# SakodaShintaro/f2-nerf

Measured on AMD Instinct MI355X. Metric: rendered rays/sec (fwd+bwd) at 800x800, higher is better.
Workload: dtype f32; 1 GPU; ngp_fox-like synthetic views 800x800, 128 samples/ray, L=16 F=2 T=2^19, 65536-ray chunks, TRAIN render + loss + backward (optimizer excluded); pixel_order=rows, regime=dense

## Files before the change

### f2-nerf_amd/csrc/host/bindings.cpp

```cpp
#include <torch/extension.h>

#include "fused_adam.hpp"
#include "hash_3d_anchored.hpp"
#include "kernel_timer.hpp"
#include "localizer.hpp"
#include "occupancy_grid.hpp"
#include "points_sampler.hpp"
#include "ragged_ops.hpp"
#include "rays.hpp"
#include "scene_files.hpp"
#include "renderer.hpp"
#include "sh_shader.hpp"

namespace py = pybind11;
using torch::Tensor;

namespace
{

torch::Device parse_device(const std::string & s)
{
  return s.empty() ? f2n::default_device() : torch::Device(s);
}

// ... 159 lines not shown
        o.step = step;
        return std::make_shared<PtsSampler>(o);
      }),
      py::arg("max_samples") = MAX_SAMPLE_PER_RAY, py::arg("step") = 1.0f / 256)
    .def(
      "get_samples",
      [](PtsSampler & s, const Tensor & o, const Tensor & d, const std::string & mode,
         const c10::optional<Tensor> & noise) {
        SampleResultFlex r = noise.has_value() ? s.get_samples(o, d, *noise)
                                               : s.get_samples(o, d, parse_mode(mode));
        return py::make_tuple(r.pts, r.dirs, r.dt, r.t, r.pts_idx_bounds);
      },
      py::arg("rays_o"), py::arg("rays_d"), py::arg("mode") = "validate",
      py::arg("noise") = py::none())
    .def(
      "get_samples_aten",
      [](PtsSampler & s, const Tensor & o, const Tensor & d, const c10::optional<Tensor> & noise) {
        SampleResultFlex r = s.get_samples_aten(o, d, opt_tensor(noise));
        return py::make_tuple(r.pts, r.dirs, r.dt, r.t, r.pts_idx_bounds);
      },
      py::arg("rays_o"), py::arg("rays_d"), py::arg("noise") = py::none());

  py::class_<SHShader, std::shared_ptr<SHShader>>(m, "SHShader")
    .def(
      py::init([](const std::string & dev) { return std::make_shared<SHShader>(parse_device(dev)); }),
      py::arg("device") = "")
    .def("query", &SHShader::query)
    .def("encode", &SHShader::encode)
    .def("named_parameters", [](SHShader & s) { return named_params(s); });

// ... 100 lines not shown
        for (auto & kv : r.named_parameters()) d[py::str(kv.key())] = grad_or_none(kv.value());
        return d;
      })
    .def(
      "set_occupancy",
      [](Renderer & r, std::shared_ptr<OccupancyGrid> g) { r.set_occupancy(std::move(g)); },
      py::arg("grid").none(true), "attach an occupancy grid (None = off): see Renderer::set_occupancy")
    .def_property_readonly("occupancy", [](Renderer & r) { return r.occupancy(); })
    .def("set_fused", [](Renderer & r, bool f) { r.options_.fused = f; })
    .def("set_fused_shade", [](Renderer & r, bool f) { r.options_.fused_shade = f; })
    .def("set_dense_first_pass", [](Renderer & r, int m) { r.options_.dense_first_pass = m; })
    .def("set_speculate_dense", [](Renderer & r, bool f) { r.options_.speculate_dense = f; })
    .def("set_pixel_tiles", [](Renderer & r, int b) { r.options_.pixel_tiles = b; })
    .def("set_fused_ray_grad", [](Renderer & r, bool f) { r.options_.fused_ray_grad = f; },
         "rays that require grad take the fused path: see RendererOptions::fused_ray_grad")
    .def("set_margin_min_samples", [](Renderer & r, int64_t n) { r.options_.margin_min_samples = n; })
    .def("set_one_pass", &Renderer::set_one_pass,
         "render_all_rays / render_image in one kernel per chunk: see RendererOptions::one_pass")
    .def("one_pass_applies", &Renderer::one_pass_applies)
    .def_property_readonly(
      "one_pass_head", [](const Renderer & r) { return r.options_.one_pass_head; },
      "RendererOptions::one_pass_head as set_one_pass_head left it")
    .def("set_one_pass_head", &Renderer::set_one_pass_head,
         "how the one-pass render walks a ray: 0 one wavefront per ray (default), -1 whole rays eight "
         "to a wavefront, a positive multiple of 64 = head then tail; see RendererOptions::one_pass_head")
    .def("set_deferred_check", [](Renderer & r, bool f) { r.options_.deferred_check = f; },
         "no host read in render(): see RendererOptions::deferred_check")
    .def("deferred_check_ok", &Renderer::deferred_check_ok)
    .def_readonly("last_kept_fraction", &Renderer::last_kept_fraction_)
    .def_readonly("last_n_samples", &Renderer::last_n_samples_)
// ... 174 lines not shown
```

### f2-nerf_amd/csrc/host/hash_3d_anchored.cpp

```cpp
#include "hash_3d_anchored.hpp"

#include "kernel_timer.hpp"

#include <cmath>

#include <c10/hip/HIPGuard.h>
#include <hip/hip_runtime_api.h>

using Tensor = torch::Tensor;

TORCH_LIBRARY(dec_hash3d_anchored, m)
{
  m.class_<Hash3DAnchoredInfo>("Hash3DAnchoredInfo").def(torch::init());
}

namespace
{

class ContractFn : public torch::autograd::Function<ContractFn>
{
public:
  static torch::autograd::variable_list forward(torch::autograd::AutogradContext * ctx, Tensor points)
  {
    points = f2n::dev_f32(points, "Hash3DAnchored::query points");
// ... 131 lines not shown
          prim_pool_.data_ptr<int32_t>(),
          bias_pool_.data_ptr<float>(),
          level_mul_.data_ptr<float>(),
          (int)options_.n_levels,
          (int)options_.n_channels,
          (uint32_t)local_size_,
          level_stride_};
}

std::pair<Tensor, Tensor> Hash3DAnchored::density_head() const
{
  return {mlp_->weight.detach().select(0, 0).contiguous(),
          mlp_->bias.detach().slice(0, 0, 1).contiguous()};
}

Tensor Hash3DAnchored::encode(const Tensor & points, int64_t samples_per_ray, Tensor * contracted_out)
{
  auto info = torch::make_intrusive<Hash3DAnchoredInfo>();
  info->hash3d_ = this;
  info->samples_per_ray_ = samples_per_ray;

  Tensor x = ContractFn::apply(points)[0];
  if (contracted_out) *contracted_out = x.detach();
  return torch::autograd::Hash3DAnchoredFunction::apply(x, feat_pool_, torch::IValue(info))[0];
}

Tensor Hash3DAnchored::encode_cached(
  const Tensor & points, const Tensor & enc_cm, const Tensor & contracted)
{
  TORCH_CHECK(
    enc_cm.dim() == 2 && enc_cm.is_contiguous() && enc_cm.size(1) == points.size(0) &&
      enc_cm.size(0) == options_.n_levels * options_.n_channels,
    "encode_cached: enc_cm must be contiguous [L*F, n]");
  auto info = torch::make_intrusive<Hash3DAnchoredInfo>();
  info->hash3d_ = this;
  info->precomputed_cm_ = enc_cm;
  const bool reuse = contracted.defined() && contracted.sizes() == points.sizes() &&
// ... 136 lines not shown
```

### f2-nerf_amd/csrc/host/hash_3d_anchored.hpp

```cpp
#pragma once

#include "common.hpp"

struct Hash3DAnchoredOptions
{
  int64_t n_levels = 16;
  int64_t n_channels = 2;
  int64_t log2_table = 19;
  int64_t level_stride = 0;
  int64_t mlp_out_dim = 16;
  bool binned_backward = true;
  bool accumulate_in_place = true;
  torch::Device device = f2n::default_device();
};

namespace f2n
{

struct FieldArgs
{
  const uint16_t * table;
  const int32_t * primes;
  const float *bias, *mul;
  int L, F;
  uint32_t T;
  int64_t level_stride;
};

}

class Hash3DAnchored : public torch::nn::Module
{
  using Tensor = torch::Tensor;

public:
  explicit Hash3DAnchored(const Hash3DAnchoredOptions & opt = {});

  Tensor query(const Tensor & points);

  Tensor encode(const Tensor & points, int64_t samples_per_ray = 0, Tensor * contracted_out = nullptr);

  Tensor encode_cached(
    const Tensor & points, const Tensor & enc_cm, const Tensor & contracted = Tensor());

  std::pair<Tensor, Tensor> density_head() const;

  Tensor table_f16();
  Tensor table_for(const Tensor & feat_pool);
  f2n::FieldArgs kernel_args(const Tensor & table16) const;

  Tensor shadow_storage();
  void mark_shadow_fresh();

  std::vector<torch::optim::OptimizerParamGroup> optim_param_groups(float lr);

// ... 40 lines not shown
```

### f2-nerf_amd/csrc/host/points_sampler.cpp

```cpp
#include "points_sampler.hpp"

using Tensor = torch::Tensor;

PtsSampler::PtsSampler(const PtsSamplerOptions & opt) : options_(opt)
{
  TORCH_CHECK(opt.max_samples >= 1 && opt.step > 0.f, "PtsSampler: bad options");
}

Tensor PtsSampler::draw_noise(int64_t n_rays, RunningMode mode, const torch::Device & device) const
{
  if (mode == RunningMode::VALIDATE) return Tensor();
  return ((torch::rand({n_rays, (int64_t)options_.max_samples}, f2n::float_on(device)) - .5f) + 1.f)
    .contiguous();
}

SampleResultFlex PtsSampler::get_samples(
  const Tensor & rays_o, const Tensor & rays_d, RunningMode mode)
{
  return get_samples(rays_o, rays_d, draw_noise(rays_o.size(0), mode, rays_o.device()));
}

SampleResultFlex PtsSampler::get_samples(
  const Tensor & rays_o_raw, const Tensor & rays_d_raw, const Tensor & noise_raw)
{
  Tensor rays_o = f2n::dev_f32(rays_o_raw, "rays_o");
  Tensor rays_d = f2n::dev_f32(rays_d_raw, "rays_d");
  const int n_rays = (int)rays_o.size(0);
  const int S = options_.max_samples;
  const int64_t n_all = (int64_t)n_rays * S;
  Tensor noise;
  if (noise_raw.defined()) {
    noise = f2n::dev_f32(noise_raw, "noise");
    TORCH_CHECK(noise.numel() == n_all, "noise must hold n_rays * max_samples values");
  }
  const auto fopt = rays_o.options();
  SampleResultFlex res;
  res.pts = torch::empty({n_all, 3}, fopt);
  res.dirs = torch::empty({n_all, 3}, fopt);
  res.dt = torch::empty({n_all}, fopt);
  res.t = torch::empty({n_all}, fopt);
  res.pts_idx_bounds = torch::empty({n_rays, 2}, f2n::int_on(rays_o.device()));
  f2n::check(
    f2n_sample_rays(
      rays_o.data_ptr<float>(), rays_d.data_ptr<float>(), f2n::fptr(noise),
      res.pts.data_ptr<float>(), res.dirs.data_ptr<float>(), res.dt.data_ptr<float>(),
      res.t.data_ptr<float>(), res.pts_idx_bounds.data_ptr<int32_t>(), n_rays, S, options_.step,
      f2n::current_stream(rays_o)),
    "f2n_sample_rays");
  return res;
}

SampleResultFlex PtsSampler::get_samples_aten(
  const Tensor & rays_o_raw, const Tensor & rays_d_raw, const Tensor & noise_raw)
{
  const int64_t S = options_.max_samples;
  Tensor rays_o = rays_o_raw.contiguous();
// ... 18 lines not shown
```

### f2-nerf_amd/csrc/host/points_sampler.hpp

```cpp
#pragma once

#include "common.hpp"

constexpr int MAX_SAMPLE_PER_RAY = 1024;

struct SampleResultFlex
{
  using Tensor = torch::Tensor;
  Tensor pts;
  Tensor dirs;
  Tensor dt;
  Tensor t;
  Tensor pts_idx_bounds;
};

enum RunningMode { TRAIN, VALIDATE };

struct PtsSamplerOptions
{
  int max_samples = MAX_SAMPLE_PER_RAY;
  float step = 1.0f / 256;
};

class PtsSampler
{
  using Tensor = torch::Tensor;

public:
  explicit PtsSampler(const PtsSamplerOptions & opt = {});

  SampleResultFlex get_samples(const Tensor & rays_o, const Tensor & rays_d, RunningMode mode);
  SampleResultFlex get_samples(const Tensor & rays_o, const Tensor & rays_d, const Tensor & noise);

  SampleResultFlex get_samples_aten(
    const Tensor & rays_o, const Tensor & rays_d, const Tensor & noise);

  Tensor draw_noise(int64_t n_rays, RunningMode mode, const torch::Device & device) const;

  PtsSamplerOptions options_;
};
```

### f2-nerf_amd/csrc/host/ragged_ops.cpp

```cpp
#include "ragged_ops.hpp"

#include "kernel_timer.hpp"

using torch::Tensor;
using torch::autograd::AutogradContext;
using torch::autograd::variable_list;

namespace
{

class FlexSumFn : public torch::autograd::Function<FlexSumFn>
{
public:
  static variable_list forward(AutogradContext * ctx, Tensor val, Tensor idx)
  {
    val = f2n::dev_f32(val, "FlexOps::Sum val");
    idx = f2n::dev_i32(idx, "FlexOps::Sum idx_start_end");
    TORCH_CHECK(val.dim() == 1 || val.dim() == 2, "FlexOps::Sum expects [n] or [n, c]");
    const int n_rays = (int)idx.size(0);
    void * s = f2n::current_stream(val);
    Tensor sum;
    if (val.dim() == 1) {
      sum = torch::empty({n_rays}, val.options());
      f2n::check(
// ... 151 lines not shown
  {
    field_out = f2n::dev_f32(field_out, "composite field_out");
    rgb = f2n::dev_f32(rgb, "composite rgb");
    dt = f2n::dev_f32(dt, "composite dt");
    t = f2n::dev_f32(t, "composite t");
    idx = f2n::dev_i32(idx, "composite idx_start_end");
    bg = f2n::dev_f32(bg, "composite bg_color");
    TORCH_CHECK(field_out.dim() == 2 && rgb.dim() == 2 && rgb.size(1) == 3, "composite shapes");
    const int64_t n = field_out.size(0);
    const int n_rays = (int)idx.size(0);
    auto opt = field_out.options();
    Tensor colors = torch::empty({n_rays, 3}, opt), depths = torch::empty({n_rays}, opt);
    Tensor weights = tiled ? torch::empty({n}, opt) : torch::zeros({n}, opt);
    Tensor last_trans = torch::empty({n_rays}, opt);
    ctx->saved_data["tiled"] = tiled;
    f2n::check(
      f2n_composite_fwd(
        f2n::fptr(field_out), field_out.size(1), f2n::fptr(rgb), f2n::fptr(dt), f2n::fptr(t),
        f2n::iptr(idx), f2n::fptr(bg), colors.data_ptr<float>(), depths.data_ptr<float>(),
        weights.data_ptr<float>(), last_trans.data_ptr<float>(), n_rays, 3.f, 1e-2f,
        f2n::current_stream(field_out)),
      "f2n_composite_fwd");
    ctx->save_for_backward({field_out, rgb, dt, t, idx, bg, weights, last_trans});
    return {colors, depths, weights};
  }

  static variable_list backward(AutogradContext * ctx, variable_list grad_output)
  {
    auto sv = ctx->get_saved_variables();
    Tensor &field_out = sv[0], &rgb = sv[1], &dt = sv[2], &t = sv[3], &idx = sv[4], &bg = sv[5],
// ... 12 lines not shown
    Tensor d_rgb = tiled ? torch::empty({n, 3}, opt) : torch::zeros({n, 3}, opt);
    f2n::check(
      f2n_composite_bwd(
        f2n::fptr(field_out), field_out.size(1), f2n::fptr(rgb), f2n::fptr(dt), f2n::fptr(t),
        f2n::iptr(idx), f2n::fptr(bg), f2n::fptr(weights), f2n::fptr(last_trans),
        f2n::fptr(d_colors), f2n::fptr(d_depths), f2n::fptr(d_weights), d_logit.data_ptr<float>(),
        d_rgb.data_ptr<float>(), n_rays, 3.f, 1e-2f, f2n::current_stream(field_out)),
      "f2n_composite_bwd");
    if (field_out.size(1) == 1)
      return {d_logit.unsqueeze(1), d_rgb, Tensor(), Tensor(), Tensor(), Tensor(), Tensor()};
    Tensor d_field = torch::zeros_like(field_out);
    d_field.select(1, 0).copy_(d_logit);
    return {d_field, d_rgb, Tensor(), Tensor(), Tensor(), Tensor(), Tensor()};
  }
};

Tensor as_channel_major(const Tensor & t)
{
  if (t.dim() == 2 && t.stride(0) == 1 && t.stride(1) == t.size(0)) return t.t();
  return t.t().contiguous();
}

class ShadeFn : public torch::autograd::Function<ShadeFn>
{
public:
  static variable_list forward(
    AutogradContext * ctx, Tensor enc, Tensor dirs, Tensor sample_img, Tensor w_h, Tensor b_h,
    Tensor w1, Tensor b1, Tensor w2, Tensor b2, Tensor app_emb)
  {
    TORCH_CHECK(enc.is_cuda() && enc.scalar_type() == torch::kFloat32 && enc.dim() == 2, "enc");
// ... 34 lines not shown

  static variable_list backward(AutogradContext * ctx, variable_list grad_output)
  {
    auto sv = ctx->get_saved_variables();
    Tensor &enc_cm = sv[0], &dirs = sv[1], &sample_img = sv[2], &w_h = sv[3], &b_h = sv[4],
           &w1 = sv[5], &b1 = sv[6], &w2 = sv[7], &b2 = sv[8], &emb = sv[9];
    const int C = (int)enc_cm.size(0);
    const int64_t n = enc_cm.size(1);
    auto opt = enc_cm.options();
    Tensor d_logit = grad_output[0].defined() ? f2n::dev_f32(grad_output[0], "d_logit")
                                              : torch::zeros({n}, opt);
    Tensor d_rgb = grad_output[1].defined() ? f2n::dev_f32(grad_output[1], "d_rgb")
                                            : torch::zeros({n, 3}, opt);
    Tensor d_enc_cm = torch::empty({(int64_t)C, n}, opt);
    const bool use_emb = emb.defined() && sample_img.defined();
    auto pad4 = [](int64_t v) { return (v + 3) / 4 * 4; };
    const int64_t sizes[7] = {w_h.numel(), b_h.numel(), w1.numel(), b1.numel(),
                              w2.numel(), b2.numel(), use_emb ? emb.numel() : 0};
    int64_t total = 0;
    for (int64_t v : sizes) total += pad4(v);
    Tensor gbuf = torch::zeros({total}, opt);
    int64_t off = 0;
    auto take = [&](const Tensor & like, int64_t numel) {
      Tensor v = gbuf.narrow(0, off, numel).view(like.sizes());
      off += pad4(numel);
      return v;
    };
    Tensor g_w_h = take(w_h, sizes[0]), g_b_h = take(b_h, sizes[1]), g_w1 = take(w1, sizes[2]),
           g_b1 = take(b1, sizes[3]), g_w2 = take(w2, sizes[4]), g_b2 = take(b2, sizes[5]);
    Tensor g_emb = use_emb ? take(emb, sizes[6]) : Tensor();
    {
    f2n::ScopedKernelTimer timer("shade_bwd", f2n::current_stream(enc_cm), (double)n);
    f2n::check(
      f2n_shade_bwd(
        enc_cm.data_ptr<float>(), C, dirs.data_ptr<float>(), use_emb ? f2n::iptr(sample_img) : nullptr,
        f2n::fptr(w_h), f2n::fptr(b_h), f2n::fptr(w1), f2n::fptr(b1), f2n::fptr(w2), f2n::fptr(b2),
        f2n::fptr(emb), f2n::fptr(d_logit), f2n::fptr(d_rgb), d_enc_cm.data_ptr<float>(),
        g_w_h.data_ptr<float>(), g_b_h.data_ptr<float>(), g_w1.data_ptr<float>(),
        g_b1.data_ptr<float>(), g_w2.data_ptr<float>(), g_b2.data_ptr<float>(),
        use_emb ? g_emb.data_ptr<float>() : nullptr, nullptr, n,
        f2n::current_stream(enc_cm)),
      "f2n_shade_bwd");
    }
    return {d_enc_cm.t(), Tensor(), Tensor(), g_w_h, g_b_h, g_w1, g_b1, g_w2, g_b2, g_emb};
  }
};

class ShadeRaysFn : public torch::autograd::Function<ShadeRaysFn>
{
public:
  static variable_list forward(
    AutogradContext * ctx, Tensor enc, Tensor dirs, Tensor ray_img, int64_t S, Tensor w_h,
    Tensor b_h, Tensor w1, Tensor b1, Tensor w2, Tensor b2, Tensor app_emb)
  {
    TORCH_CHECK(enc.is_cuda() && enc.scalar_type() == torch::kFloat32 && enc.dim() == 2, "enc");
    const int64_t n = enc.size(0);
    const int C = (int)enc.size(1);
    TORCH_CHECK(S > 0 && S % 64 == 0 && n % S == 0 && n < ((int64_t)1 << 28), "shade_rays: n = n_rays * S, S % 64 == 0");
    const int n_rays = (int)(n / S);
// ... 36 lines not shown

  static variable_list backward(AutogradContext * ctx, variable_list grad_output)
  {
    auto sv = ctx->get_saved_variables();
    Tensor &enc_cm = sv[0], &dirs = sv[1], &ray_img = sv[2], &w_h = sv[3], &b_h = sv[4],
           &w1 = sv[5], &b1 = sv[6], &w2 = sv[7], &b2 = sv[8], &emb = sv[9];
    const int C = (int)enc_cm.size(0);
    const int64_t n = enc_cm.size(1), S = ctx->saved_data["S"].toInt();
    auto opt = enc_cm.options();
    Tensor d_logit = grad_output[0].defined() ? f2n::dev_f32(grad_output[0], "d_logit")
                                              : torch::zeros({n}, opt);
    Tensor d_rgb = grad_output[1].defined() ? f2n::dev_f32(grad_output[1], "d_rgb")
                                            : torch::zeros({n, 3}, opt);
    Tensor d_enc_cm = torch::empty({(int64_t)C, n}, opt);
    const bool use_emb = emb.defined() && ray_img.defined();
    auto pad4 = [](int64_t v) { return (v + 3) / 4 * 4; };
    const int64_t sizes[7] = {w_h.numel(), b_h.numel(), w1.numel(), b1.numel(),
                              w2.numel(), b2.numel(), use_emb ? emb.numel() : 0};
    int64_t total = 0;
    for (int64_t v : sizes) total += pad4(v);
    Tensor gbuf = torch::zeros({total}, opt);
    int64_t off = 0;
    auto take = [&](const Tensor & like, int64_t numel) {
      Tensor v = gbuf.narrow(0, off, numel).view(like.sizes());
      off += pad4(numel);
      return v;
    };
    Tensor g_w_h = take(w_h, sizes[0]), g_b_h = take(b_h, sizes[1]), g_w1 = take(w1, sizes[2]),
           g_b1 = take(b1, sizes[3]), g_w2 = take(w2, sizes[4]), g_b2 = take(b2, sizes[5]);
    Tensor g_emb = use_emb ? take(emb, sizes[6]) : Tensor();
    {
    f2n::ScopedKernelTimer timer("shade_bwd", f2n::current_stream(enc_cm), (double)n);
    f2n::check(
      f2n_shade_bwd_rays(
        enc_cm.data_ptr<float>(), C, dirs.data_ptr<float>(), use_emb ? f2n::iptr(ray_img) : nullptr,
        f2n::fptr(w_h), f2n::fptr(b_h), f2n::fptr(w1), f2n::fptr(b1), f2n::fptr(w2), f2n::fptr(b2),
        f2n::fptr(emb), f2n::fptr(d_logit), f2n::fptr(d_rgb), d_enc_cm.data_ptr<float>(),
        g_w_h.data_ptr<float>(), g_b_h.data_ptr<float>(), g_w1.data_ptr<float>(),
        g_b1.data_ptr<float>(), g_w2.data_ptr<float>(), g_b2.data_ptr<float>(),
        use_emb ? g_emb.data_ptr<float>() : nullptr, (int)(n / S), (int)S,
        f2n::current_stream(enc_cm)),
      "f2n_shade_bwd_rays");
    }
    return {d_enc_cm.t(), Tensor(), Tensor(), Tensor(), g_w_h, g_b_h, g_w1, g_b1, g_w2, g_b2, g_emb};
  }
};


class TrainLossFn : public torch::autograd::Function<TrainLossFn>
{
public:
  static variable_list forward(
    AutogradContext * ctx, Tensor colors, Tensor gt, Tensor var, double var_weight)
  {
    colors = f2n::dev_f32(colors, "train_loss colors");
    gt = f2n::dev_f32(gt, "train_loss gt_colors");
    var = f2n::dev_f32(var, "train_loss var");
    const int64_t n_rays = colors.size(0);
    TORCH_CHECK(
// ... 105 lines not shown
bool f2n::shade_rays_applies(int64_t n, int64_t n_rays, int64_t S)
{
  return n_rays > 0 && S > 0 && S % 64 == 0 && n == n_rays * S && n < ((int64_t)1 << 28) &&
         f2n_get_option(F2N_OPT_SHADE_RAYS) == 0 && f2n_get_option(F2N_OPT_SHADE_FWD) == 0 &&
         f2n_get_option(F2N_OPT_SHADE_BWD) == 0;
}

f2n::CompositeOut f2n::composite(
  const Tensor & field_out, const Tensor & rgb, const Tensor & dt, const Tensor & t,
  const Tensor & idx_start_end, const Tensor & bg_color, bool bounds_tile_samples)
{
  auto out = CompositeFn::apply(field_out, rgb, dt, t, idx_start_end, bg_color, bounds_tile_samples);
  return {out[0], out[1], out[2]};
}

Tensor f2n::train_loss(
  const Tensor & colors, const Tensor & gt_colors, const Tensor & var, float var_loss_weight)
{
  return TrainLossFn::apply(colors, gt_colors, var, (double)var_loss_weight)[0];
}
```

### f2-nerf_amd/csrc/host/ragged_ops.hpp

```cpp
#pragma once

#include "common.hpp"

namespace torch::autograd
{

class TruncExp : public Function<TruncExp>
{
public:
  static variable_list forward(AutogradContext * ctx, Tensor input);
  static variable_list backward(AutogradContext * ctx, variable_list grad_output);
};

}

namespace FlexOps
{
torch::Tensor Sum(torch::Tensor val, torch::Tensor idx_start_end);
torch::Tensor AccumulateSum(torch::Tensor val, torch::Tensor idx_start_end, bool include_this);
}

namespace CustomOps
{
torch::Tensor WeightVar(torch::Tensor weights, torch::Tensor idx_start_end);
// ... 25 lines not shown
ShadeOut shade(
  const Tensor & enc, const Tensor & dirs, const Tensor & sample_img, const Tensor & w_h,
  const Tensor & b_h, const Tensor & w1, const Tensor & b1, const Tensor & w2, const Tensor & b2,
  const Tensor & app_emb);

ShadeOut shade_rays(
  const Tensor & enc, const Tensor & dirs, const Tensor & ray_img, int64_t S, const Tensor & w_h,
  const Tensor & b_h, const Tensor & w1, const Tensor & b1, const Tensor & w2, const Tensor & b2,
  const Tensor & app_emb);

bool shade_rays_applies(int64_t n, int64_t n_rays, int64_t S);

Tensor train_loss(
  const Tensor & colors, const Tensor & gt_colors, const Tensor & var, float var_loss_weight);

inline bool shade_supported(int64_t C) { return C == 8 || C == 16 || C == 32 || C == 64; }

}
```

### f2-nerf_amd/csrc/host/renderer.cpp

```cpp
#include "renderer.hpp"

#include "kernel_timer.hpp"

#include "ragged_ops.hpp"
#include "rays.hpp"

#include <c10/hip/HIPGuard.h>
#include <hip/hip_runtime_api.h>

using Tensor = torch::Tensor;

f2n::HostCount::~HostCount()
{
  if (event_) hipEventDestroy((hipEvent_t)event_);
  if (pinned_) hipHostFree(pinned_);
}

void f2n::HostCount::request(const torch::Tensor & device_int32, void * stream)
{
  TORCH_CHECK(
    device_int32.is_cuda() && device_int32.scalar_type() == torch::kInt32 && device_int32.numel() == 1,
    "HostCount: one int32 on the device");
  const int device = (int)device_int32.device().index();
  c10::hip::HIPGuard on_device(device);
// ... 46 lines not shown
class RayUnpermuteFn : public torch::autograd::Function<RayUnpermuteFn>
{
public:
  static torch::autograd::variable_list forward(
    torch::autograd::AutogradContext * ctx, Tensor colors, Tensor depths, Tensor weights,
    Tensor perm, Tensor inv, Tensor bounds_sorted, Tensor bounds_caller, int64_t S, bool rows)
  {
    colors = f2n::dev_f32(colors, "colors");
    depths = f2n::dev_f32(depths, "depths");
    weights = f2n::dev_f32(weights, "weights");
    const int n = (int)perm.size(0);
    void * s = f2n::current_stream(colors);
    Tensor c = torch::empty_like(colors), d = torch::empty_like(depths), w = torch::empty_like(weights);
    gather(colors, depths, weights, c, d, w, inv, bounds_sorted, bounds_caller, n, S, rows, s);
    ctx->save_for_backward({perm, bounds_sorted, bounds_caller});
    ctx->saved_data["S"] = S;
    ctx->saved_data["rows"] = rows;
    return {c, d, w};
  }

  static torch::autograd::variable_list backward(
    torch::autograd::AutogradContext * ctx, torch::autograd::variable_list g)
  {
    auto saved = ctx->get_saved_variables();
    const Tensor & perm = saved[0];
    const int n = (int)perm.size(0);
    const int64_t S = ctx->saved_data["S"].toInt();
    const bool rows = ctx->saved_data["rows"].toBool();
    Tensor gc = g[0].defined() ? f2n::dev_f32(g[0], "grad colors") : Tensor();
    Tensor gd = g[1].defined() ? f2n::dev_f32(g[1], "grad depths") : Tensor();
// ... 332 lines not shown
    bounds = bounds_from_counts(counts, stream).first;
  }
  auto out = RayUnpermuteFn::apply(
    r.colors, r.depths, r.weights, perm, inv, r.idx_start_end, bounds, S, rows);
  return {out[0], out[1], out[2], bounds};
}

RenderResult Renderer::render_dense(
  const Tensor & rays_o, const Tensor & rays_d, const Tensor & emb_idx, RunningMode mode,
  const Tensor & noise, const Tensor & bg_color, const Route & route)
{
  const int n_rays = (int)rays_o.size(0);
  const int S = pts_sampler_->options_.max_samples;
  void * stream = f2n::current_stream(rays_o);
  Hash3DAnchored & field = *scene_field_;
  SampleResultFlex all = pts_sampler_->get_samples(rays_o, rays_d, noise);
  const int64_t n_all = all.pts.size(0);
  Tensor contracted_all, enc_all_cm;
  {
    torch::NoGradGuard no_grad;
    enc_all_cm = field.encode(all.pts, S, &contracted_all).t();
    TORCH_CHECK(enc_all_cm.is_contiguous(), "encode() must return channel-major storage");
  }

  if (options_.deferred_check) {
    Tensor total = scan_survivors(all, enc_all_cm, n_rays).second;
    if (!deferred_bad_.defined()) deferred_bad_ = torch::zeros({1}, total.options());
    deferred_bad_.add_(total.ne(n_all).to(torch::kInt32));
    record_kept(n_all, n_all);
    return shade_and_composite(all, emb_idx, mode, bg_color, route, enc_all_cm, contracted_all);
  }

  const bool may_guess = options_.speculate_dense && last_kept_fraction_ >= 1.f && n_all > 0;
  const bool large = n_all >= options_.margin_min_samples;
  if (may_guess && large) {
    if (auto guess = shade_all_unless_near_threshold(
// ... 362 lines not shown
  Renderer & renderer, const Tensor & rays_o, const Tensor & rays_d, const Tensor & emb_idx,
  const Tensor & gt_colors, float var_loss_weight, const Tensor & noise, const Tensor & bg_color,
  bool run_backward)
{
  RenderResult res =
    renderer.render(rays_o, rays_d, emb_idx, RunningMode::TRAIN, noise, bg_color);
  Tensor var = CustomOps::WeightVar(res.weights, res.idx_start_end);
  if (var_loss_weight == 0.f) var = var.detach();
  Tensor stats = f2n::train_loss(res.colors, gt_colors, var, var_loss_weight);
  Tensor loss = stats[0];
  TrainStepResult out;
  out.loss = loss.detach();
  out.sq_err_sum = stats[3].detach();
  out.n_values = res.colors.numel();
  out.n_samples = renderer.last_n_samples_;
  if (run_backward && loss.requires_grad()) loss.backward();
  return out;
}
```

### f2-nerf_amd/csrc/kernels/sampler.hip

```cpp
#include "hash_grid.hiph"
#include "occupancy.hiph"
#include "sampler.hiph"

namespace
{

__device__ __forceinline__ int ray_of_wave()
{
  return (int)blockIdx.x * F2N_WAVES_PER_BLOCK + (int)(threadIdx.x >> 6);
}


__global__ __launch_bounds__(F2N_BLOCK) void sample_rays_kernel(
  const float * __restrict__ rays_o, const float * __restrict__ rays_d,
  const float * __restrict__ noise, float * __restrict__ pts, float * __restrict__ dirs,
  float * __restrict__ dt, float * __restrict__ t, int32_t * __restrict__ bounds, int n_rays, int S,
  float step)
{
  const int r = ray_of_wave();
  if (r >= n_rays) return;
  const int lane = lane_id();
  const RayFrame rf = load_ray(rays_o, rays_d, r);
  const float * nrow = noise ? noise + (int64_t)r * S : nullptr;
  StrideCarry carry = {0.f, 0.f, 0.f, 0.f};
  const int64_t base = (int64_t)r * S;
  for (int k0 = 0; k0 < S; k0 += F2N_WAVE) {
    const StrideSample sm = make_stride(rf, nrow, k0, S, step, carry, lane);
    if (sm.valid) {
      const int64_t i = base + k0 + lane;
      pts[3 * i] = sm.px;
      pts[3 * i + 1] = sm.py;
      pts[3 * i + 2] = sm.pz;
      dirs[3 * i] = rf.dx;
      dirs[3 * i + 1] = rf.dy;
      dirs[3 * i + 2] = rf.dz;
      dt[i] = sm.dt;
      t[i] = sm.t;
    }
  }
  if (lane == 0) {
    bounds[2 * r] = (int32_t)base;
    bounds[2 * r + 1] = (int32_t)(base + S);
  }
}


__global__ __launch_bounds__(F2N_BLOCK) void sample_compact_kernel(
  const float * __restrict__ rays_o, const float * __restrict__ rays_d,
  const float * __restrict__ noise, const int32_t * __restrict__ bounds, float * __restrict__ pts,
  float * __restrict__ dirs, float * __restrict__ dt, float * __restrict__ t, int n_rays, int S,
  float step)
{
  const int r = ray_of_wave();
  if (r >= n_rays) return;
  const int lane = lane_id();
  const int start = bounds[2 * r];
  const int cnt = bounds[2 * r + 1] - start;
// ... 539 lines not shown
  }
  if (total && blockIdx.x == gridDim.x - 1 && tid == 0) total[0] = offset + all;
}

}

extern "C" int f2n_sample_rays(
  const float * rays_o, const float * rays_d, const float * noise, float * pts, float * dirs,
  float * dt, float * t, int32_t * bounds, int n_rays, int S, float step, void * stream)
{
  if (n_rays < 0 || S < 1) return F2N_E_INVALID_ARG;
  if ((int64_t)n_rays * S > INT32_MAX) return F2N_E_INVALID_ARG;
  if (n_rays == 0) return F2N_OK;
  if (!rays_o || !rays_d || !pts || !dirs || !dt || !t || !bounds) return F2N_E_INVALID_ARG;
  hipLaunchKernelGGL(
    sample_rays_kernel, dim3(f2n_div_up(n_rays, F2N_WAVES_PER_BLOCK)), dim3(F2N_BLOCK), 0,
    (hipStream_t)stream, rays_o, rays_d, noise, pts, dirs, dt, t, bounds, n_rays, S, step);
  return f2n_launch_status();
}

extern "C" int f2n_sample_compact(
  const float * rays_o, const float * rays_d, const float * noise, const int32_t * bounds,
  float * pts, float * dirs, float * dt, float * t, int n_rays, int S, float step, void * stream)
{
  if (n_rays < 0 || S < 1) return F2N_E_INVALID_ARG;
  if (n_rays == 0) return F2N_OK;
  if (!rays_o || !rays_d || !bounds) return F2N_E_INVALID_ARG;
  hipLaunchKernelGGL(
    sample_compact_kernel, dim3(f2n_div_up(n_rays, F2N_WAVES_PER_BLOCK)), dim3(F2N_BLOCK), 0,
    (hipStream_t)stream, rays_o, rays_d, noise, bounds, pts, dirs, dt, t, n_rays, S, step);
  return f2n_launch_status();
}
// ... 147 lines not shown
```

### f2-nerf_amd/csrc/kernels/status.hip

```cpp
#include "common.hiph"

#include <atomic>

namespace
{
std::atomic<int> g_options[F2N_OPT_COUNT];

bool option_value_ok(int key, int value)
{
  switch (key) {
    case F2N_OPT_SHADE_FWD:
    case F2N_OPT_SHADE_BWD:
    case F2N_OPT_BWD_COMBINE:
    case F2N_OPT_BWD_PHASES:
    case F2N_OPT_RAY_ORDER:
    case F2N_OPT_SHADE_RAYS: return value == 0 || value == 1;
    case F2N_OPT_MARCH: return value >= 0 && value <= 2;
    case F2N_OPT_SHADE_BWD_WAVES: return value >= 0 && value <= 3;
    case F2N_OPT_SHADE_VARIANT: return value >= 0 && value <= 3;
    case F2N_OPT_RAYTILE: return value == 0 || value == 16 || value == 32;
    case F2N_OPT_HASH_BWD: return value >= 0 && value <= 2;
    case F2N_OPT_RAYTILE_WALK: return value >= 0 && value <= 3;
    default: return false;
  }
}
}

extern "C" int f2n_set_option(int key, int value)
{
  if (key < 0 || key >= F2N_OPT_COUNT || !option_value_ok(key, value)) return F2N_E_INVALID_ARG;
  return g_options[key].exchange(value, std::memory_order_relaxed);
// ... 21 lines not shown
```

### include/f2nerf_hip.h

```cpp
#ifndef F2NERF_HIP_H_
#define F2NERF_HIP_H_

#include <stdint.h>

#ifdef __cplusplus
extern "C" {
#endif

#define F2N_ABI_VERSION 2

#define F2N_OK 0
#define F2N_E_INVALID_ARG (-1)
#define F2N_E_LAUNCH (-2)
#define F2N_E_UNSUPPORTED (-3)

#define F2N_MAX_LEVELS 32

int f2n_abi_version(void);
const char * f2n_status_string(int status);

#define F2N_OPT_SHADE_FWD 0
#define F2N_OPT_SHADE_BWD 1
#define F2N_OPT_SHADE_VARIANT 2
#define F2N_OPT_RAYTILE 3
#define F2N_OPT_HASH_BWD 4
#define F2N_OPT_BWD_COMBINE 5
#define F2N_OPT_RAYTILE_WALK 6
#define F2N_OPT_MARCH 7
#define F2N_OPT_BWD_PHASES 8
#define F2N_OPT_RAY_ORDER 9
#define F2N_OPT_SHADE_BWD_WAVES 10
#define F2N_SHADE_BWD_TWO_WAVES_MIN_SAMPLES (3 << 19)
#define F2N_OPT_SHADE_RAYS 11
#define F2N_OPT_COUNT 12
int f2n_set_option(int key, int value);
int f2n_get_option(int key);


int f2n_table_to_f16(const float * table_f32, uint16_t * table_f16, int64_t n, void * stream);

int f2n_hash_fwd(
  const float * pts, const uint16_t * table_f16, const int32_t * primes, const float * bias,
  const float * mul, float * out, int64_t out_ld_point, int64_t out_ld_chan, uint32_t * idx_out,
  int64_t n, int L, int F, uint32_t T, int64_t level_stride, void * stream);

int f2n_hash_fwd_raytile(
  const float * pts, const uint16_t * table_f16, const int32_t * primes, const float * bias,
  const float * mul, float * out_cm, int n_rays, int S, int L, int F, uint32_t T,
  int64_t level_stride, void * stream);
// ... 72 lines not shown
  float * rays_d, int64_t n, void * stream);

int f2n_gen_rays_dist_bwd(
  const float * intrinsics, const float * dist, int64_t n_cams, const int32_t * ij,
  int64_t first_pixel, int width, const float * d_rays_o, const float * d_rays_d, float * d_poses,
  int pose_ld, float * workspace, int64_t n, void * stream);

int f2n_project_points(
  const float * points, const float * poses, int pose_ld, const float * intrinsics,
  const float * dist, int64_t n_cams, const int32_t * cam_idx, float * pix, int32_t * valid,
  int64_t n, void * stream);

int f2n_sample_rays(
  const float * rays_o, const float * rays_d, const float * noise, float * pts, float * dirs,
  float * dt, float * t, int32_t * bounds, int n_rays, int S, float step, void * stream);

int f2n_density_march(
  const float * rays_o, const float * rays_d, const float * noise, const uint16_t * table_f16,
  const int32_t * primes, const float * bias, const float * mul, const float * w0, const float * b0,
  int32_t * kept, int n_rays, int S, float step, int L, int F, uint32_t T, int64_t level_stride,
  float t_thresh, float density_shift, void * stream);

int f2n_density_scan(
  const float * enc_cm, int C, const float * dt, const float * w0, const float * b0, int32_t * kept,
  int n_rays, int S, float t_thresh, float density_shift, void * stream);

int f2n_density_margin(
  const float * logit, const float * dt, int32_t * flag, int n_rays, int S, float density_shift,
  float depth_limit, void * stream);

// ... 157 lines not shown
```

Measured before the change: 12.34 million rays/s.

## Fuse contraction into sampler, in-place net grads, fused noise offset

Three unrelated speedups are bundled. The sampler kernel can now also write contracted points, so the hash encode skips its separate contract pass in the dense path. Network parameter gradients are accumulated directly into existing .grad buffers during train-step backward, which avoids a zeroed scratch allocation and the later accumulation. Random noise is offset with one vectorized kernel instead of two elementwise torch ops, and materialize_grads is turned off on two autograd functions. These add option flags and aliasing complexity, and writing gradients in place risks wrong accumulation semantics.

```diff
diff --git a/f2-nerf_amd/csrc/host/bindings.cpp b/f2-nerf_amd/csrc/host/bindings.cpp
--- a/f2-nerf_amd/csrc/host/bindings.cpp
+++ b/f2-nerf_amd/csrc/host/bindings.cpp
@@ -197,6 +197,15 @@
       py::arg("rays_o"), py::arg("rays_d"), py::arg("mode") = "validate",
       py::arg("noise") = py::none())
     .def(
+      "draw_noise",
+      [](PtsSampler & s, int64_t n_rays, const std::string & mode,
+         const std::string & dev) -> c10::optional<Tensor> {
+        Tensor noise = s.draw_noise(n_rays, parse_mode(mode), parse_device(dev));
+        return noise.defined() ? c10::optional<Tensor>(noise) : c10::nullopt;
+      },
+      py::arg("n_rays"), py::arg("mode") = "train", py::arg("device") = "",
+      "the step noise get_samples(mode) draws: [n_rays, max_samples] in TRAIN, None in VALIDATE")
+    .def(
       "get_samples_aten",
       [](PtsSampler & s, const Tensor & o, const Tensor & d, const c10::optional<Tensor> & noise) {
         SampleResultFlex r = s.get_samples_aten(o, d, opt_tensor(noise));
@@ -327,6 +336,8 @@
     .def("set_pixel_tiles", [](Renderer & r, int b) { r.options_.pixel_tiles = b; })
     .def("set_fused_ray_grad", [](Renderer & r, bool f) { r.options_.fused_ray_grad = f; },
          "rays that require grad take the fused path: see RendererOptions::fused_ray_grad")
+    .def("set_ray_order_min_rays", [](Renderer & r, int64_t n) { r.options_.ray_order_min_rays = n; },
+         "rays per chunk from which the dense first pass buckets them: see RendererOptions")
     .def("set_margin_min_samples", [](Renderer & r, int64_t n) { r.options_.margin_min_samples = n; })
     .def("set_one_pass", &Renderer::set_one_pass,
          "render_all_rays / render_image in one kernel per chunk: see RendererOptions::one_pass")
diff --git a/f2-nerf_amd/csrc/host/hash_3d_anchored.cpp b/f2-nerf_amd/csrc/host/hash_3d_anchored.cpp
--- a/f2-nerf_amd/csrc/host/hash_3d_anchored.cpp
+++ b/f2-nerf_amd/csrc/host/hash_3d_anchored.cpp
@@ -169,13 +169,16 @@
           mlp_->bias.detach().slice(0, 0, 1).contiguous()};
 }
 
-Tensor Hash3DAnchored::encode(const Tensor & points, int64_t samples_per_ray, Tensor * contracted_out)
+Tensor Hash3DAnchored::encode(
+  const Tensor & points, int64_t samples_per_ray, Tensor * contracted_out, const Tensor & contracted)
 {
   auto info = torch::make_intrusive<Hash3DAnchoredInfo>();
   info->hash3d_ = this;
   info->samples_per_ray_ = samples_per_ray;
 
-  Tensor x = ContractFn::apply(points)[0];
+  const bool reuse = contracted.defined() && contracted.sizes() == points.sizes() &&
+                     !(torch::GradMode::is_enabled() && points.requires_grad());
+  Tensor x = reuse ? contracted : ContractFn::apply(points)[0];
   if (contracted_out) *contracted_out = x.detach();
   return torch::autograd::Hash3DAnchoredFunction::apply(x, feat_pool_, torch::IValue(info))[0];
 }
diff --git a/f2-nerf_amd/csrc/host/hash_3d_anchored.hpp b/f2-nerf_amd/csrc/host/hash_3d_anchored.hpp
--- a/f2-nerf_amd/csrc/host/hash_3d_anchored.hpp
+++ b/f2-nerf_amd/csrc/host/hash_3d_anchored.hpp
@@ -38,7 +38,9 @@
 
   Tensor query(const Tensor & points);
 
-  Tensor encode(const Tensor & points, int64_t samples_per_ray = 0, Tensor * contracted_out = nullptr);
+  Tensor encode(
+    const Tensor & points, int64_t samples_per_ray = 0, Tensor * contracted_out = nullptr,
+    const Tensor & contracted = Tensor());
 
   Tensor encode_cached(
     const Tensor & points, const Tensor & enc_cm, const Tensor & contracted = Tensor());
diff --git a/f2-nerf_amd/csrc/host/points_sampler.cpp b/f2-nerf_amd/csrc/host/points_sampler.cpp
--- a/f2-nerf_amd/csrc/host/points_sampler.cpp
+++ b/f2-nerf_amd/csrc/host/points_sampler.cpp
@@ -10,8 +10,11 @@
 Tensor PtsSampler::draw_noise(int64_t n_rays, RunningMode mode, const torch::Device & device) const
 {
   if (mode == RunningMode::VALIDATE) return Tensor();
-  return ((torch::rand({n_rays, (int64_t)options_.max_samples}, f2n::float_on(device)) - .5f) + 1.f)
-    .contiguous();
+  Tensor u = torch::rand({n_rays, (int64_t)options_.max_samples}, f2n::float_on(device));
+  if (!u.is_cuda()) return ((u - .5f) + 1.f).contiguous();
+  f2n::check(
+    f2n_noise_offset(u.data_ptr<float>(), u.numel(), f2n::current_stream(u)), "f2n_noise_offset");
+  return u;
 }
 
 SampleResultFlex PtsSampler::get_samples(
@@ -21,7 +24,8 @@
 }
 
 SampleResultFlex PtsSampler::get_samples(
-  const Tensor & rays_o_raw, const Tensor & rays_d_raw, const Tensor & noise_raw)
+  const Tensor & rays_o_raw, const Tensor & rays_d_raw, const Tensor & noise_raw,
+  Tensor * contracted_out)
 {
   Tensor rays_o = f2n::dev_f32(rays_o_raw, "rays_o");
   Tensor rays_d = f2n::dev_f32(rays_d_raw, "rays_d");
@@ -40,6 +44,17 @@
   res.dt = torch::empty({n_all}, fopt);
   res.t = torch::empty({n_all}, fopt);
   res.pts_idx_bounds = torch::empty({n_rays, 2}, f2n::int_on(rays_o.device()));
+  if (contracted_out && f2n_get_option(F2N_OPT_SAMPLE_CONTRACT) == 0) {
+    *contracted_out = torch::empty({n_all, 3}, fopt);
+    f2n::check(
+      f2n_sample_rays_contracted(
+        rays_o.data_ptr<float>(), rays_d.data_ptr<float>(), f2n::fptr(noise),
+        res.pts.data_ptr<float>(), contracted_out->data_ptr<float>(), res.dirs.data_ptr<float>(),
+        res.dt.data_ptr<float>(), res.t.data_ptr<float>(), res.pts_idx_bounds.data_ptr<int32_t>(),
+        n_rays, S, options_.step, f2n::current_stream(rays_o)),
+      "f2n_sample_rays_contracted");
+    return res;
+  }
   f2n::check(
     f2n_sample_rays(
       rays_o.data_ptr<float>(), rays_d.data_ptr<float>(), f2n::fptr(noise),
diff --git a/f2-nerf_amd/csrc/host/points_sampler.hpp b/f2-nerf_amd/csrc/host/points_sampler.hpp
--- a/f2-nerf_amd/csrc/host/points_sampler.hpp
+++ b/f2-nerf_amd/csrc/host/points_sampler.hpp
@@ -30,7 +30,9 @@
   explicit PtsSampler(const PtsSamplerOptions & opt = {});
 
   SampleResultFlex get_samples(const Tensor & rays_o, const Tensor & rays_d, RunningMode mode);
-  SampleResultFlex get_samples(const Tensor & rays_o, const Tensor & rays_d, const Tensor & noise);
+  SampleResultFlex get_samples(
+    const Tensor & rays_o, const Tensor & rays_d, const Tensor & noise,
+    Tensor * contracted_out = nullptr);
 
   SampleResultFlex get_samples_aten(
     const Tensor & rays_o, const Tensor & rays_d, const Tensor & noise);
diff --git a/f2-nerf_amd/csrc/host/ragged_ops.cpp b/f2-nerf_amd/csrc/host/ragged_ops.cpp
--- a/f2-nerf_amd/csrc/host/ragged_ops.cpp
+++ b/f2-nerf_amd/csrc/host/ragged_ops.cpp
@@ -1,6 +1,9 @@
 #include "ragged_ops.hpp"
 
 #include "kernel_timer.hpp"
+
+#include <array>
+#include <atomic>
 
 using torch::Tensor;
 using torch::autograd::AutogradContext;
@@ -189,6 +192,7 @@
     Tensor weights = tiled ? torch::empty({n}, opt) : torch::zeros({n}, opt);
     Tensor last_trans = torch::empty({n_rays}, opt);
     ctx->saved_data["tiled"] = tiled;
+    ctx->set_materialize_grads(false);
     f2n::check(
       f2n_composite_fwd(
         f2n::fptr(field_out), field_out.size(1), f2n::fptr(rgb), f2n::fptr(dt), f2n::fptr(t),
@@ -231,6 +235,51 @@
     return {d_field, d_rgb, Tensor(), Tensor(), Tensor(), Tensor(), Tensor()};
   }
 };
+
+std::atomic<bool> g_net_grad_in_place{false};
+
+struct NetGrads
+{
+  Tensor buf[7];
+  bool in_place[7];
+  Tensor out(int i) const { return in_place[i] ? Tensor() : buf[i]; }
+};
+
+NetGrads net_grad_buffers(
+  AutogradContext * ctx, std::array<const Tensor *, 7> params, int first_input, bool use_emb)
+{
+  NetGrads g;
+  const bool may = g_net_grad_in_place.load(std::memory_order_relaxed) &&
+                   f2n_get_option(F2N_OPT_NET_GRAD_IN_PLACE) == 0 && !torch::GradMode::is_enabled();
+  auto pad4 = [](int64_t v) { return (v + 3) / 4 * 4; };
+  int64_t total = 0;
+  for (int i = 0; i < 7; i++) {
+    g.in_place[i] = false;
+    if (i == 6 && !use_emb) continue;
+    const Tensor & p = *params[i];
+    if (may && p.is_leaf() && ctx->needs_input_grad(first_input + i)) {
+      const Tensor & have = p.grad();
+      if (have.defined() && have.is_contiguous() && have.scalar_type() == torch::kFloat32 &&
+          have.device() == p.device() && have.sizes() == p.sizes() &&
+          reinterpret_cast<uintptr_t>(have.data_ptr()) % 16 == 0) {
+        g.buf[i] = have;
+        g.in_place[i] = true;
+        continue;
+      }
+    }
+    total += pad4(p.numel());
+  }
+  if (total == 0) return g;
+  Tensor gbuf = torch::zeros({total}, params[0]->options());
+  int64_t off = 0;
+  for (int i = 0; i < 7; i++) {
+    if (g.in_place[i] || (i == 6 && !use_emb)) continue;
+    const Tensor & p = *params[i];
+    g.buf[i] = gbuf.narrow(0, off, p.numel()).view(p.sizes());
+    off += pad4(p.numel());
+  }
+  return g;
+}
 
 Tensor as_channel_major(const Tensor & t)
 {
@@ -295,21 +344,9 @@
                                             : torch::zeros({n, 3}, opt);
     Tensor d_enc_cm = torch::empty({(int64_t)C, n}, opt);
     const bool use_emb = emb.defined() && sample_img.defined();
-    auto pad4 = [](int64_t v) { return (v + 3) / 4 * 4; };
-    const int64_t sizes[7] = {w_h.numel(), b_h.numel(), w1.numel(), b1.numel(),
-                              w2.numel(), b2.numel(), use_emb ? emb.numel() : 0};
-    int64_t total = 0;
-    for (int64_t v : sizes) total += pad4(v);
-    Tensor gbuf = torch::zeros({total}, opt);
-    int64_t off = 0;
-    auto take = [&](const Tensor & like, int64_t numel) {
-      Tensor v = gbuf.narrow(0, off, numel).view(like.sizes());
-      off += pad4(numel);
-      return v;
-    };
-    Tensor g_w_h = take(w_h, sizes[0]), g_b_h = take(b_h, sizes[1]), g_w1 = take(w1, sizes[2]),
-           g_b1 = take(b1, sizes[3]), g_w2 = take(w2, sizes[4]), g_b2 = take(b2, sizes[5]);
-    Tensor g_emb = use_emb ? take(emb, sizes[6]) : Tensor();
+    const NetGrads g = net_grad_buffers(ctx, {&w_h, &b_h, &w1, &b1, &w2, &b2, &emb}, 3, use_emb);
+    const Tensor &g_w_h = g.buf[0], &g_b_h = g.buf[1], &g_w1 = g.buf[2], &g_b1 = g.buf[3],
+                 &g_w2 = g.buf[4], &g_b2 = g.buf[5], &g_emb = g.buf[6];
     {
     f2n::ScopedKernelTimer timer("shade_bwd", f2n::current_stream(enc_cm), (double)n);
     f2n::check(
@@ -323,7 +360,8 @@
         f2n::current_stream(enc_cm)),
       "f2n_shade_bwd");
     }
-    return {d_enc_cm.t(), Tensor(), Tensor(), g_w_h, g_b_h, g_w1, g_b1, g_w2, g_b2, g_emb};
+    return {d_enc_cm.t(), Tensor(), Tensor(), g.out(0), g.out(1), g.out(2), g.out(3), g.out(4),
+            g.out(5), g.out(6)};
   }
 };
 
@@ -390,21 +428,9 @@
                                             : torch::zeros({n, 3}, opt);
     Tensor d_enc_cm = torch::empty({(int64_t)C, n}, opt);
     const bool use_emb = emb.defined() && ray_img.defined();
-    auto pad4 = [](int64_t v) { return (v + 3) / 4 * 4; };
-    const int64_t sizes[7] = {w_h.numel(), b_h.numel(), w1.numel(), b1.numel(),
-                              w2.numel(), b2.numel(), use_emb ? emb.numel() : 0};
-    int64_t total = 0;
-    for (int64_t v : sizes) total += pad4(v);
-    Tensor gbuf = torch::zeros({total}, opt);
-    int64_t off = 0;
-    auto take = [&](const Tensor & like, int64_t numel) {
-      Tensor v = gbuf.narrow(0, off, numel).view(like.sizes());
-      off += pad4(numel);
-      return v;
-    };
-    Tensor g_w_h = take(w_h, sizes[0]), g_b_h = take(b_h, sizes[1]), g_w1 = take(w1, sizes[2]),
-           g_b1 = take(b1, sizes[3]), g_w2 = take(w2, sizes[4]), g_b2 = take(b2, sizes[5]);
-    Tensor g_emb = use_emb ? take(emb, sizes[6]) : Tensor();
+    const NetGrads g = net_grad_buffers(ctx, {&w_h, &b_h, &w1, &b1, &w2, &b2, &emb}, 3, use_emb);
+    const Tensor &g_w_h = g.buf[0], &g_b_h = g.buf[1], &g_w1 = g.buf[2], &g_b1 = g.buf[3],
+                 &g_w2 = g.buf[4], &g_b2 = g.buf[5], &g_emb = g.buf[6];
     {
     f2n::ScopedKernelTimer timer("shade_bwd", f2n::current_stream(enc_cm), (double)n);
     f2n::check(
@@ -418,7 +444,8 @@
         f2n::current_stream(enc_cm)),
       "f2n_shade_bwd_rays");
     }
-    return {d_enc_cm.t(), Tensor(), Tensor(), Tensor(), g_w_h, g_b_h, g_w1, g_b1, g_w2, g_b2, g_emb};
+    return {d_enc_cm.t(), Tensor(), Tensor(), Tensor(), g.out(0), g.out(1), g.out(2), g.out(3),
+            g.out(4), g.out(5), g.out(6)};
   }
 };
 
@@ -554,6 +581,9 @@
   return {out[0], out[1], out[2]};
 }
 
+f2n::NetGradInPlaceScope::NetGradInPlaceScope() : prev_(g_net_grad_in_place.exchange(true)) {}
+f2n::NetGradInPlaceScope::~NetGradInPlaceScope() { g_net_grad_in_place.store(prev_); }
+
 Tensor f2n::train_loss(
   const Tensor & colors, const Tensor & gt_colors, const Tensor & var, float var_loss_weight)
 {
diff --git a/f2-nerf_amd/csrc/host/ragged_ops.hpp b/f2-nerf_amd/csrc/host/ragged_ops.hpp
--- a/f2-nerf_amd/csrc/host/ragged_ops.hpp
+++ b/f2-nerf_amd/csrc/host/ragged_ops.hpp
@@ -63,6 +63,18 @@
 Tensor train_loss(
   const Tensor & colors, const Tensor & gt_colors, const Tensor & var, float var_loss_weight);
 
+class NetGradInPlaceScope
+{
+public:
+  NetGradInPlaceScope();
+  ~NetGradInPlaceScope();
+  NetGradInPlaceScope(const NetGradInPlaceScope &) = delete;
+  NetGradInPlaceScope & operator=(const NetGradInPlaceScope &) = delete;
+
+private:
+  bool prev_;
+};
+
 inline bool shade_supported(int64_t C) { return C == 8 || C == 16 || C == 32 || C == 64; }
 
 }
diff --git a/f2-nerf_amd/csrc/host/renderer.cpp b/f2-nerf_amd/csrc/host/renderer.cpp
--- a/f2-nerf_amd/csrc/host/renderer.cpp
+++ b/f2-nerf_amd/csrc/host/renderer.cpp
@@ -84,6 +84,7 @@
     Tensor c = torch::empty_like(colors), d = torch::empty_like(depths), w = torch::empty_like(weights);
     gather(colors, depths, weights, c, d, w, inv, bounds_sorted, bounds_caller, n, S, rows, s);
     ctx->save_for_backward({perm, bounds_sorted, bounds_caller});
+    ctx->set_materialize_grads(false);
     ctx->saved_data["S"] = S;
     ctx->saved_data["rows"] = rows;
     return {c, d, w};
@@ -446,12 +447,14 @@
   const int S = pts_sampler_->options_.max_samples;
   void * stream = f2n::current_stream(rays_o);
   Hash3DAnchored & field = *scene_field_;
-  SampleResultFlex all = pts_sampler_->get_samples(rays_o, rays_d, noise);
+  Tensor sampler_contracted;
+  SampleResultFlex all = pts_sampler_->get_samples(rays_o, rays_d, noise, &sampler_contracted);
   const int64_t n_all = all.pts.size(0);
   Tensor contracted_all, enc_all_cm;
   {
     torch::NoGradGuard no_grad;
-    enc_all_cm = field.encode(all.pts, S, &contracted_all).t();
+    enc_all_cm =
+      field.encode(all.pts, S, &contracted_all, sampler_contracted).t();
     TORCH_CHECK(enc_all_cm.is_contiguous(), "encode() must return channel-major storage");
   }
 
@@ -844,6 +847,9 @@
   out.sq_err_sum = stats[3].detach();
   out.n_values = res.colors.numel();
   out.n_samples = renderer.last_n_samples_;
-  if (run_backward && loss.requires_grad()) loss.backward();
+  if (run_backward && loss.requires_grad()) {
+    f2n::NetGradInPlaceScope in_place;
+    loss.backward();
+  }
   return out;
 }
diff --git a/f2-nerf_amd/csrc/kernels/sampler.hip b/f2-nerf_amd/csrc/kernels/sampler.hip
--- a/f2-nerf_amd/csrc/kernels/sampler.hip
+++ b/f2-nerf_amd/csrc/kernels/sampler.hip
@@ -11,11 +11,12 @@
 }
 
 
+template <bool CONTRACTED>
 __global__ __launch_bounds__(F2N_BLOCK) void sample_rays_kernel(
   const float * __restrict__ rays_o, const float * __restrict__ rays_d,
-  const float * __restrict__ noise, float * __restrict__ pts, float * __restrict__ dirs,
-  float * __restrict__ dt, float * __restrict__ t, int32_t * __restrict__ bounds, int n_rays, int S,
-  float step)
+  const float * __restrict__ noise, float * __restrict__ pts, float * __restrict__ xc,
+  float * __restrict__ dirs, float * __restrict__ dt, float * __restrict__ t,
+  int32_t * __restrict__ bounds, int n_rays, int S, float step)
 {
   const int r = ray_of_wave();
   if (r >= n_rays) return;
@@ -31,6 +32,13 @@
       pts[3 * i] = sm.px;
       pts[3 * i + 1] = sm.py;
       pts[3 * i + 2] = sm.pz;
+      if constexpr (CONTRACTED) {
+        float x = sm.px, y = sm.py, z = sm.pz;
+        contract_point(x, y, z);
+        xc[3 * i] = x;
+        xc[3 * i + 1] = y;
+        xc[3 * i + 2] = z;
+      }
       dirs[3 * i] = rf.dx;
       dirs[3 * i + 1] = rf.dy;
       dirs[3 * i + 2] = rf.dz;
@@ -41,6 +49,21 @@
   if (lane == 0) {
     bounds[2 * r] = (int32_t)base;
     bounds[2 * r + 1] = (int32_t)(base + S);
+  }
+}
+
+__global__ __launch_bounds__(F2N_BLOCK) void noise_offset_kernel(float * __restrict__ u, int64_t n)
+{
+  const int64_t i = ((int64_t)blockIdx.x * F2N_BLOCK + threadIdx.x) * 4;
+  if (i + 4 <= n && (reinterpret_cast<uintptr_t>(u) & 15u) == 0) {
+    float4 v = *reinterpret_cast<float4 *>(u + i);
+    v.x = __fadd_rn(__fsub_rn(v.x, .5f), 1.f);
+    v.y = __fadd_rn(__fsub_rn(v.y, .5f), 1.f);
+    v.z = __fadd_rn(__fsub_rn(v.z, .5f), 1.f);
+    v.w = __fadd_rn(__fsub_rn(v.w, .5f), 1.f);
+    *reinterpret_cast<float4 *>(u + i) = v;
+  } else {
+    for (int64_t j = i; j < n && j < i + 4; j++) u[j] = __fadd_rn(__fsub_rn(u[j], .5f), 1.f);
   }
 }
 
@@ -610,8 +633,35 @@
   if (n_rays == 0) return F2N_OK;
   if (!rays_o || !rays_d || !pts || !dirs || !dt || !t || !bounds) return F2N_E_INVALID_ARG;
   hipLaunchKernelGGL(
-    sample_rays_kernel, dim3(f2n_div_up(n_rays, F2N_WAVES_PER_BLOCK)), dim3(F2N_BLOCK), 0,
-    (hipStream_t)stream, rays_o, rays_d, noise, pts, dirs, dt, t, bounds, n_rays, S, step);
+    sample_rays_kernel<false>, dim3(f2n_div_up(n_rays, F2N_WAVES_PER_BLOCK)), dim3(F2N_BLOCK), 0,
+    (hipStream_t)stream, rays_o, rays_d, noise, pts, (float *)nullptr, dirs, dt, t, bounds, n_rays,
+    S, step);
+  return f2n_launch_status();
+}
+
+extern "C" int f2n_sample_rays_contracted(
+  const float * rays_o, const float * rays_d, const float * noise, float * pts, float * x,
+  float * dirs, float * dt, float * t, int32_t * bounds, int n_rays, int S, float step,
+  void * stream)
+{
+  if (n_rays < 0 || S < 1) return F2N_E_INVALID_ARG;
+  if ((int64_t)n_rays * S > INT32_MAX) return F2N_E_INVALID_ARG;
+  if (n_rays == 0) return F2N_OK;
+  if (!rays_o || !rays_d || !pts || !x || !dirs || !dt || !t || !bounds) return F2N_E_INVALID_ARG;
+  hipLaunchKernelGGL(
+    sample_rays_kernel<true>, dim3(f2n_div_up(n_rays, F2N_WAVES_PER_BLOCK)), dim3(F2N_BLOCK), 0,
+    (hipStream_t)stream, rays_o, rays_d, noise, pts, x, dirs, dt, t, bounds, n_rays, S, step);
+  return f2n_launch_status();
+}
+
+extern "C" int f2n_noise_offset(float * u, int64_t n, void * stream)
+{
+  if (n < 0 || n > ((int64_t)1 << 40)) return F2N_E_INVALID_ARG;
+  if (n == 0) return F2N_OK;
+  if (!u) return F2N_E_INVALID_ARG;
+  hipLaunchKernelGGL(
+    noise_offset_kernel, dim3(f2n_div_up(f2n_div_up(n, 4), F2N_BLOCK)), dim3(F2N_BLOCK), 0,
+    (hipStream_t)stream, u, n);
   return f2n_launch_status();
 }
 
diff --git a/f2-nerf_amd/csrc/kernels/status.hip b/f2-nerf_amd/csrc/kernels/status.hip
--- a/f2-nerf_amd/csrc/kernels/status.hip
+++ b/f2-nerf_amd/csrc/kernels/status.hip
@@ -14,7 +14,9 @@
     case F2N_OPT_BWD_COMBINE:
     case F2N_OPT_BWD_PHASES:
     case F2N_OPT_RAY_ORDER:
-    case F2N_OPT_SHADE_RAYS: return value == 0 || value == 1;
+    case F2N_OPT_SHADE_RAYS:
+    case F2N_OPT_NET_GRAD_IN_PLACE:
+    case F2N_OPT_SAMPLE_CONTRACT: return value == 0 || value == 1;
     case F2N_OPT_MARCH: return value >= 0 && value <= 2;
     case F2N_OPT_SHADE_BWD_WAVES: return value >= 0 && value <= 3;
     case F2N_OPT_SHADE_VARIANT: return value >= 0 && value <= 3;
diff --git a/include/f2nerf_hip.h b/include/f2nerf_hip.h
--- a/include/f2nerf_hip.h
+++ b/include/f2nerf_hip.h
@@ -32,7 +32,9 @@
 #define F2N_OPT_SHADE_BWD_WAVES 10
 #define F2N_SHADE_BWD_TWO_WAVES_MIN_SAMPLES (3 << 19)
 #define F2N_OPT_SHADE_RAYS 11
-#define F2N_OPT_COUNT 12
+#define F2N_OPT_NET_GRAD_IN_PLACE 12
+#define F2N_OPT_SAMPLE_CONTRACT 13
+#define F2N_OPT_COUNT 14
 int f2n_set_option(int key, int value);
 int f2n_get_option(int key);
 
@@ -135,6 +137,13 @@
 int f2n_sample_rays(
   const float * rays_o, const float * rays_d, const float * noise, float * pts, float * dirs,
   float * dt, float * t, int32_t * bounds, int n_rays, int S, float step, void * stream);
+
+int f2n_sample_rays_contracted(
+  const float * rays_o, const float * rays_d, const float * noise, float * pts, float * x,
+  float * dirs, float * dt, float * t, int32_t * bounds, int n_rays, int S, float step,
+  void * stream);
+
+int f2n_noise_offset(float * u, int64_t n, void * stream);
 
 int f2n_density_march(
   const float * rays_o, const float * rays_d, const float * noise, const uint16_t * table_f16,
```

Measured after the change: 12.48 million rays/s (median of 5 runs). 1.2% higher.
